# LiWentomng/OrientedRepPoints

Measured on NVIDIA H100. Metric: 1024x1024 tiles/sec, higher is better.
Workload: dtype f16x3

## Files before the change

### orientedreppoints_b200/csrc/dense_tc.cu

```cuda
#include <cuda.h>
#include <cuda_bf16.h>
#include <cuda_fp16.h>

#include <mutex>
#include <type_traits>

#include "common.cuh"
#include "../../include/orp_b200_group.h"
#include "wgmma.cuh"

namespace orp {
namespace {

constexpr int kMaxProb = 5;
constexpr int kStagesMax = 6;
constexpr int kBM = 128;
constexpr int kBK = 64;
constexpr int kABytes = kBM * kBK * 2;

struct FastDiv {
    uint32_t mul, shr, d;
    __host__ void set(uint32_t div)
    {
        d = div;
        uint32_t l = 0;
        while ((1ull << l) < div) ++l;
        shr = l;
        mul = (uint32_t)(((1ull << 32) * ((1ull << l) - div)) / div + 1);
    }
    __device__ __forceinline__ uint32_t div(uint32_t n) const { return (__umulhi(n, mul) + n) >> shr; }
    __device__ __forceinline__ void divmod(uint32_t n, uint32_t &q, uint32_t &r) const { q = div(n); r = n - q * d; }
};

struct Problem {
    int N, H, W, Ho, Wo;
    FastDiv fd_tw, fd_th;
    int BW, BH, BI;
    int lbw, lbh;
    int tiles_w, tiles_h, tiles_i, tile_start;
    void *out;
    const __nv_bfloat16 *res;
    const float *res32;
    const __nv_bfloat16 *x;
    const float *offset;
    const float *mask;
    double *gn_stats;
};

struct alignas(64) TcParams {
    CUtensorMap tmA[kMaxProb];
    CUtensorMap tmB;
    CUtensorMap tmOut[kMaxProb];
    CUtensorMap tmRes[kMaxProb];
    CUtensorMap tmI;
    Problem prob[kMaxProb];
    int tma_epi, epi_bufs;
    int epi_merge;
    int ncat;
    int ksplit;
    FastDiv fd_ks;
    long long ks_stride;
    int b_resident;
    int res_mma;
    int gn_fused;
    int dcat;
    int split;
    float oscale;
    unsigned int *ovf;
    int nprob, num_m_tiles, n_tiles_n, num_tiles;
    FastDiv fd_ntn;
    int KH, KW, Cin, cin_blocks, stride, pad, Cout, relu;
    int s2d_stem;
    const float *bias;
    int gw;
};

__device__ __forceinline__ uint32_t smem_u32(const void *p) { return (uint32_t)__cvta_generic_to_shared(p); }

__device__ __forceinline__ void mbar_init(uint64_t *bar, uint32_t count)
{
    asm volatile("mbarrier.init.shared::cta.b64 [%0], %1;" ::"r"(smem_u32(bar)), "r"(count));
}
__device__ __forceinline__ void mbar_expect_tx(uint64_t *bar, uint32_t bytes)
{
    asm volatile("mbarrier.arrive.expect_tx.shared::cta.b64 _, [%0], %1;" ::"r"(smem_u32(bar)), "r"(bytes) : "memory");
}
// ... 907 lines not shown
                                const float vy = wv.x * f1.y + wv.y * f2.y + wv.z * f3.y + wv.w * f4.y;
                                __nv_bfloat162 b2 = __floats2bfloat162_rn(vx, vy);
                                pk[k] = *reinterpret_cast<uint32_t *>(&b2);
                            }
                            *reinterpret_cast<uint4 *>(sa + (size_t)row * 128 + ((c16 ^ (row & 7)) << 4)) = make_uint4(pk[0], pk[1], pk[2], pk[3]);
                        }
                        asm volatile("fence.proxy.async.shared::cta;" ::: "memory");
                        __syncwarp();
                        if ((pt & 31) == 0) mbar_arrive(&full[r.stage]);
                        r.next();
                    } else {
                        const __half *xh = reinterpret_cast<const __half *>(pr.x);
                        auto load_item = [&](int it, uint4 (&u)[4][2]) {
                            const int item = pt + it * kDP, row = item >> 3, c16 = item & 7;
                            const int4 ov = s_o[tb][row];
                            const int co = cb * kBK + c16 * 8;
                            const int oo[4] = {ov.x, ov.y, ov.z, ov.w};
#pragma unroll
                            for (int c = 0; c < 4; ++c) {
                                u[c][0] = *reinterpret_cast<const uint4 *>(xh + oo[c] + co);
                                u[c][1] = *reinterpret_cast<const uint4 *>(xh + oo[c] + P.Cin + co);
                            }
                        };
                        auto item_at = [&](int it) {
                            const int item = pt + it * kDP, row = item >> 3, c16 = item & 7;
                            return (uint32_t)(row * 128 + ((c16 ^ (row & 7)) << 4));
                        };
                        if constexpr (!kFragEpi) {
                            uint32_t phi[kDItems][4], plo[kDItems][4];
#pragma unroll
                            for (int i2 = 0; i2 < kDItems / kDRound; ++i2) {
                                uint4 u[kDRound][4][2];
#pragma unroll
                                for (int i1 = 0; i1 < kDRound; ++i1) load_item(i2 * kDRound + i1, u[i1]);
#pragma unroll
                                for (int i1 = 0; i1 < kDRound; ++i1) {
                                    const int it = i2 * kDRound + i1, row = (pt + it * kDP) >> 3;
                                    split_sample(u[i1], s_w[tb][row], s_wh[tb][row], phi[it], plo[it]);
                                }
                            }
                            mbar_wait(&empty[r.stage], r.phase ^ 1);
                            if (pt == 0) load_b(r.stage, tap, cb, nt);
                            uint8_t *sa = smem + (size_t)r.stage * kStageBytes;
#pragma unroll
                            for (int it = 0; it < kDItems; ++it) {
                                const uint32_t at = item_at(it);
                                *reinterpret_cast<uint4 *>(sa + at) = make_uint4(phi[it][0], phi[it][1], phi[it][2], phi[it][3]);
                                *reinterpret_cast<uint4 *>(sa + kABytes + at) = make_uint4(plo[it][0], plo[it][1], plo[it][2], plo[it][3]);
                            }
                        } else {
                            const uint32_t sa = smem_u32(smem + (size_t)r.stage * kStageBytes);
#pragma unroll
                            for (int i2 = 0; i2 < kDItems / kDRound; ++i2) {
                                uint4 u[kDRound][4][2];
#pragma unroll
                                for (int i1 = 0; i1 < kDRound; ++i1) load_item(i2 * kDRound + i1, u[i1]);
                                if (i2 == 0) {
                                    mbar_wait(&empty[r.stage], r.phase ^ 1);
                                    if (pt == 0) load_b(r.stage, tap, cb, nt);
                                }
#pragma unroll
                                for (int i1 = 0; i1 < kDRound; ++i1) {
                                    const int it = i2 * kDRound + i1, row = (pt + it * kDP) >> 3;
                                    uint32_t hi[4], lo[4];
                                    split_sample(u[i1], s_w[tb][row], s_wh[tb][row], hi, lo);
                                    const uint32_t at = sa + item_at(it);
                                    sts128(at, make_uint4(hi[0], hi[1], hi[2], hi[3]));
                                    sts128(at + kABytes, make_uint4(lo[0], lo[1], lo[2], lo[3]));
                                }
                            }
                        }
                        asm volatile("fence.proxy.async.shared::cta;" ::: "memory");
                        __syncwarp();
                        if ((pt & 31) == 0) mbar_arrive(&full[r.stage]);
                        r.next();
                    }
                }
                tb ^= 1;
            }
        }
    }
}

typedef CUresult (*EncodeTiledFn)(CUtensorMap *, CUtensorMapDataType, cuuint32_t, void *, const cuuint64_t *, const cuuint64_t *,
                                  const cuuint32_t *, const cuuint32_t *, CUtensorMapInterleave, CUtensorMapSwizzle,
                                  CUtensorMapL2promotion, CUtensorMapFloatOOBfill);

EncodeTiledFn encode_fn()
{
    static EncodeTiledFn fn = nullptr;
    static std::once_flag once;
    std::call_once(once, [] {
        void *p = nullptr;
        cudaDriverEntryPointQueryResult st;
        if (cudaGetDriverEntryPoint("cuTensorMapEncodeTiled", &p, cudaEnableDefault, &st) == cudaSuccess && st == cudaDriverEntryPointSuccess)
            fn = reinterpret_cast<EncodeTiledFn>(p);
    });
    return fn;
}

int pow2_floor(int v) { int p = 1; while (p * 2 <= v) p *= 2; return p; }

constexpr int kEvPool = 1024;
thread_local cudaEvent_t g_tc_ev[kEvPool][2];
thread_local int g_tc_ev_created = 0, g_tc_ev_used = 0;
thread_local double g_tc_flops = 0.0;
thread_local orp_tc_plan g_tc_plan;
thread_local bool g_tc_plan_set = false;

constexpr int kSmemPerBlock = 227 * 1024;
constexpr int kStaticSmemPlain = 4096;
constexpr int kStaticSmemDeform = 14336;

struct ConvDesc {
    int nprob;
    const orp_tc_problem *probs;
    const void *w;
    int Cout, Cout_padded, KH, KW, Cin, stride, pad;
    const float *bias;
    int relu, out_f32, deform;
    int split;
    int wscale_log2;
    int stem;
    int ksplit;
    int gw;
};

struct ConvPlan {
    orp_tc_plan rep;
    Problem prob[kMaxProb];
    int num_m_tiles;
    int kbn;
    int extra_bytes;
};

int check_conv(const ConvDesc &d)
{
    if (d.split && (d.wscale_log2 < 0 || d.wscale_log2 > 15)) return fail(ORP_EINVAL, "conv2d_f16x3: weight scale exponent must be in 0..15");
    if (d.nprob < 1 || d.nprob > kMaxProb || !d.probs || !d.w) return fail(ORP_EINVAL, "conv2d_tc: bad arguments");
    if (d.Cin % 8) return fail(ORP_EINVAL, "conv2d_tc: Cin must be a multiple of 8 (16-byte channel rows)");
    if (d.deform && (d.Cin % kBK)) return fail(ORP_EINVAL, "conv2d_tc: deformable conv needs Cin % 64 == 0");
    if (d.Cout_padded % 32 || d.Cout_padded < d.Cout) return fail(ORP_EINVAL, "conv2d_tc: padded Cout must be a multiple of 32");
    if (d.stride < 1 || d.stride > 256) return fail(ORP_EINVAL, "conv2d_tc: stride must be in 1..256");
    if (d.deform)
        for (int i = 0; i < d.nprob; ++i)
            if ((long long)d.probs[i].N * d.probs[i].H * d.probs[i].W * d.Cin * (d.split ? 2 : 1) >= (1LL << 31))
                return fail(ORP_EINVAL, "conv2d_tc: deformable input has 2^31 or more 16-bit elements (32-bit sample offsets)");
    const orp_tc_problem &q0 = d.probs[0];
    if (d.ksplit > 1 && (d.nprob != 1 || d.deform || d.stem || !d.out_f32 || (d.KH * d.KW) % d.ksplit || q0.residual_bf16 ||
                         q0.residual_f32 || d.bias || d.relu))
        return fail(ORP_EINVAL, "conv2d_tc: split-K serves one plain problem with an fp32 partial-sum output and taps % ksplit == 0");
    if (d.gw) {
        if (d.gw != 4 && d.gw != 8 && d.gw != 16 && d.gw != 32 && d.gw != 64)
            return fail(ORP_EINVAL, "group_conv2d: group width (width / groups) must be 4, 8, 16, 32 or 64");
        if (d.Cout % kBK || d.Cin != d.Cout || d.Cout_padded != d.Cout)
            return fail(ORP_EINVAL, "group_conv2d: width must be a multiple of 64");
        if (d.nprob != 1 || d.out_f32 || d.deform || d.stem || d.ksplit != 1 || d.relu == 2 || d.KH != 3 || d.KW != 3 || d.pad != 1 ||
            q0.residual_bf16 || q0.residual_f32 || q0.offset || q0.mask || q0.gn_stats)
            return fail(ORP_EINVAL, "group_conv2d: one 3x3 / pad 1 problem with a 16-bit output; no residual, fp32 output, GroupNorm "
                                    "statistics, deformation or split-K");
    }
    return ORP_OK;
}

int plan_conv(const ConvDesc &d, int sms, ConvPlan &pl)
{
// ... 56 lines not shown
    int epi_bufs = mem_bound ? 2 : 1;
    const int epi_merge = (d.split && tma_epi && !frag_epi && (mem_bound || d.stem == 2)) ? 1 : 0;
    const int dcat = (d.split && d.deform) ? 1 : 0;
    const int ncat = (d.split && tma_epi && BN <= 128 && !d.deform && !any_res && !d.gw) ? 1 : 0;
    const int res_mma = (tma_epi && any_res) ? 1 : 0;
    if (res_mma) {
        if (d.deform) return fail(ORP_EINVAL, "conv2d_tc: residual is not supported on the deformable path");
        for (int i = 0; i < nprob; ++i)
            if (!probs[i].residual_bf16) return fail(ORP_EINVAL, "conv2d_tc: residual must be given for every problem or none");
    }
    const int slab_bytes = d.KH * d.KW * T * cin_blocks * BN * kBK * 2;
    int b_resident = (!d.deform && ksplit == 1 && slab_bytes <= 72 * 1024) ? 1 : 0;
    int grid = num_tiles / n_pair < sms ? num_tiles / n_pair : sms;
    if (b_resident && grid >= n_tiles_n) grid -= grid % n_tiles_n;
    else if (b_resident) b_resident = 0;
    int stage_b = 0, extra = 0, stages = 0;
    for (;;) {
        stage_b = stage_bytes(kbn, ncat || dcat, b_resident);
        const int hc = BN < 64 ? BN : 64;
        int staging = d.out_f32 ? 0 : 128 * (hc * 2 + 16);
        if (tma_epi) staging = epi_bufs * (epi_merge ? 32768 : 16384);
        extra = (res_mma ? 8192 : 0) + (b_resident ? slab_bytes : 0) + staging;
        stages = (kSmemPerBlock - (d.deform ? kStaticSmemDeform : kStaticSmemPlain) - dyn_smem_bytes(stage_b, 0, extra, frag_epi)) / stage_b;
        if (stages >= 3) break;
        if (epi_bufs == 2) { epi_bufs = 1; continue; }
        if (b_resident) { b_resident = 0; continue; }
        if (stages >= 2) break;
        return fail(ORP_EINVAL, "conv2d_tc: shared-memory budget cannot hold two main-loop stages");
    }
    if (stages > kStagesMax) stages = kStagesMax;
    if (d.deform && stages > 3) stages = 3;

    pl.num_m_tiles = mt;
    pl.kbn = kbn;
    pl.extra_bytes = extra;
    orp_tc_plan &r = pl.rep;
    r.BN = BN; r.stages = stages; r.grid = grid; r.num_tiles = num_tiles; r.n_tiles_n = n_tiles_n;
    r.ksplit = ksplit; r.nprob = nprob; r.Cout = d.Cout; r.Cout_padded = d.Cout_padded;
    r.split = d.split ? 1 : 0; r.deform = d.deform ? 1 : 0; r.out_f32 = d.out_f32 ? 1 : 0; r.stem = d.stem; r.relu = d.relu;
    r.bias = d.bias ? 1 : 0;
    for (int i = 0; i < nprob; ++i) {
        if (probs[i].residual_bf16) r.residual = 1;
        else if (probs[i].residual_f32) r.residual = 2;
        r.BW[i] = pl.prob[i].BW; r.BH[i] = pl.prob[i].BH; r.BI[i] = pl.prob[i].BI;
    }
    r.tma_epi = tma_epi; r.ncat = ncat; r.dcat = dcat; r.res_mma = res_mma; r.b_resident = b_resident;
    r.epi_merge = epi_merge; r.epi_bufs = epi_bufs; r.gn_fused = gn_fused; r.n_pair = n_pair;
    return ORP_OK;
}

int make_params(const ConvDesc &d, const ConvPlan &pl, TcParams &P)
{
    memset(&P, 0, sizeof(P));
    P.nprob = d.nprob; P.KH = d.KH; P.KW = d.KW; P.Cin = d.Cin; P.cin_blocks = d.gw ? 1 : (d.Cin + kBK - 1) / kBK;
    P.gw = d.gw;
    P.stride = d.stride; P.pad = d.pad;
    P.Cout = d.Cout; P.relu = d.relu; P.bias = d.bias; P.s2d_stem = (d.stem == 2) ? 1 : 0;
    P.split = d.split ? 1 : 0;
    P.oscale = d.split ? ldexpf(1.f, -d.wscale_log2) : 1.f;
    {
        void *ovf = nullptr;
        ORP_CUDA(cudaGetSymbolAddress(&ovf, g_f16_overflow));
        P.ovf = static_cast<unsigned int *>(ovf);
    }
    P.n_tiles_n = pl.rep.n_tiles_n / pl.rep.n_pair;
    P.fd_ntn.set((uint32_t)P.n_tiles_n);
    for (int i = 0; i < d.nprob; ++i) {
        const orp_tc_problem &q = d.probs[i];
        Problem &pr = P.prob[i];
        pr = pl.prob[i];
        pr.out = q.out; pr.res = static_cast<const __nv_bfloat16 *>(q.residual_bf16); pr.res32 = q.residual_f32;
        pr.x = static_cast<const __nv_bfloat16 *>(q.x); pr.offset = q.offset; pr.gn_stats = q.gn_stats; pr.mask = q.mask;
    }
    P.num_m_tiles = pl.num_m_tiles;
    P.num_tiles = pl.rep.num_tiles / pl.rep.n_pair;
    P.ksplit = d.ksplit;
    P.fd_ks.set((uint32_t)d.ksplit);
    P.ks_stride = (long long)P.prob[0].N * P.prob[0].Ho * P.prob[0].Wo * d.Cout;
    P.tma_epi = pl.rep.tma_epi; P.epi_bufs = pl.rep.epi_bufs; P.epi_merge = pl.rep.epi_merge; P.ncat = pl.rep.ncat;
    P.b_resident = pl.rep.b_resident; P.res_mma = pl.rep.res_mma; P.gn_fused = pl.rep.gn_fused; P.dcat = pl.rep.dcat;
    return ORP_OK;
}

int encode_maps(const ConvDesc &d, const ConvPlan &pl, TcParams &P)
{
    EncodeTiledFn enc = encode_fn();
    if (!enc) return fail(ORP_ECUDA, "conv2d_tc: cuTensorMapEncodeTiled unavailable");
    const CUtensorMapDataType dt16 = d.split ? CU_TENSOR_MAP_DATA_TYPE_FLOAT16 : CU_TENSOR_MAP_DATA_TYPE_BFLOAT16;
    const int T = d.split ? 2 : 1, Cin = d.Cin, Cout = d.Cout, stride = d.stride;
    if (!d.deform) {
        for (int i = 0; i < d.nprob; ++i) {
            const orp_tc_problem &q = d.probs[i];
            const Problem &pr = P.prob[i];
            cuuint64_t gdim[5] = {(cuuint64_t)Cin, (cuuint64_t)T, (cuuint64_t)q.W, (cuuint64_t)q.H, (cuuint64_t)q.N};
            cuuint64_t gstr[4] = {(cuuint64_t)Cin * 2, (cuuint64_t)Cin * 2 * T, (cuuint64_t)q.W * Cin * 2 * T,
                                  (cuuint64_t)q.H * q.W * Cin * 2 * T};
            if (d.stem == 2) {
                gstr[0] = (cuuint64_t)q.N * q.H * (q.W + 3) * 32;
                gstr[1] = 32;
                gstr[2] = (cuuint64_t)(q.W + 3) * 32;
                gstr[3] = (cuuint64_t)q.H * (q.W + 3) * 32;
            }
            cuuint32_t box[5] = {(cuuint32_t)kBK, 1u, (cuuint32_t)(pr.BW * stride), (cuuint32_t)(pr.BH * stride), (cuuint32_t)pr.BI};
            cuuint32_t estr[5] = {1, 1, (cuuint32_t)stride, (cuuint32_t)stride, 1};
            CUresult r = enc(&P.tmA[i], dt16, 5, const_cast<void *>(q.x), gdim, gstr, box, estr,
                             CU_TENSOR_MAP_INTERLEAVE_NONE, CU_TENSOR_MAP_SWIZZLE_128B, CU_TENSOR_MAP_L2_PROMOTION_L2_128B,
                             CU_TENSOR_MAP_FLOAT_OOB_FILL_NONE);
            if (r != CUDA_SUCCESS) return fail(ORP_ECUDA, "conv2d_tc: cuTensorMapEncodeTiled(A) failed");
        }
    }
    {
        const cuuint64_t K = (cuuint64_t)d.KH * d.KW * T * P.cin_blocks * kBK;
        cuuint64_t gdim[2] = {K, (cuuint64_t)d.Cout_padded};
        cuuint64_t gstr[1] = {K * 2};
        cuuint32_t box[2] = {(cuuint32_t)kBK, (cuuint32_t)pl.kbn};
        cuuint32_t estr[2] = {1, 1};
        CUresult r = enc(&P.tmB, dt16, 2, const_cast<void *>(d.w), gdim, gstr, box, estr,
                         CU_TENSOR_MAP_INTERLEAVE_NONE, CU_TENSOR_MAP_SWIZZLE_128B, CU_TENSOR_MAP_L2_PROMOTION_L2_256B,
                         CU_TENSOR_MAP_FLOAT_OOB_FILL_NONE);
        if (r != CUDA_SUCCESS) return fail(ORP_ECUDA, "conv2d_tc: cuTensorMapEncodeTiled(B) failed");
    }
    if (P.res_mma) {
        void *ident_ptr = nullptr;
        if (d.split) {
            ORP_CUDA(cudaGetSymbolAddress(&ident_ptr, g_ident16));
            ident_ptr = static_cast<char *>(ident_ptr) + (size_t)d.wscale_log2 * 8192;
        } else {
            ORP_CUDA(cudaGetSymbolAddress(&ident_ptr, g_ident));
        }
        cuuint64_t gdim[2] = {64, 64};
        cuuint64_t gstr[1] = {128};
        cuuint32_t box[2] = {64, 64};
        cuuint32_t estr[2] = {1, 1};
        CUresult r = enc(&P.tmI, dt16, 2, ident_ptr, gdim, gstr, box, estr, CU_TENSOR_MAP_INTERLEAVE_NONE,
                         CU_TENSOR_MAP_SWIZZLE_128B, CU_TENSOR_MAP_L2_PROMOTION_NONE, CU_TENSOR_MAP_FLOAT_OOB_FILL_NONE);
        if (r != CUDA_SUCCESS) return fail(ORP_ECUDA, "conv2d_tc: cuTensorMapEncodeTiled(identity) failed");
    }
    if (P.tma_epi) {
        for (int i = 0; i < d.nprob; ++i) {
            const Problem &pr = P.prob[i];
            cuuint64_t gdim[5] = {(cuuint64_t)Cout, (cuuint64_t)T, (cuuint64_t)pr.Wo, (cuuint64_t)pr.Ho, (cuuint64_t)pr.N};
            cuuint64_t gstr[4] = {(cuuint64_t)Cout * 2, (cuuint64_t)Cout * 2 * T, (cuuint64_t)pr.Wo * Cout * 2 * T,
                                  (cuuint64_t)pr.Ho * pr.Wo * Cout * 2 * T};
            cuuint32_t box[5] = {64u, 1u, (cuuint32_t)pr.BW, (cuuint32_t)pr.BH, (cuuint32_t)pr.BI};
            cuuint32_t estr[5] = {1, 1, 1, 1, 1};
            CUresult r = enc(&P.tmOut[i], dt16, 5, pr.out, gdim, gstr, box, estr,
                             CU_TENSOR_MAP_INTERLEAVE_NONE, CU_TENSOR_MAP_SWIZZLE_128B, CU_TENSOR_MAP_L2_PROMOTION_NONE,
                             CU_TENSOR_MAP_FLOAT_OOB_FILL_NONE);
            if (r != CUDA_SUCCESS) return fail(ORP_ECUDA, "conv2d_tc: cuTensorMapEncodeTiled(out) failed");
            if (pr.res) {
                r = enc(&P.tmRes[i], dt16, 5, const_cast<__nv_bfloat16 *>(pr.res), gdim, gstr, box, estr,
                        CU_TENSOR_MAP_INTERLEAVE_NONE, CU_TENSOR_MAP_SWIZZLE_128B, CU_TENSOR_MAP_L2_PROMOTION_L2_128B,
                        CU_TENSOR_MAP_FLOAT_OOB_FILL_NONE);
                if (r != CUDA_SUCCESS) return fail(ORP_ECUDA, "conv2d_tc: cuTensorMapEncodeTiled(residual) failed");
            }
        }
    }
    return ORP_OK;
}

template <int BN, bool OUT_F32, bool DEFORM, bool SPLIT, int WALK>
int launch_tc(const TcParams &P, int stages, int grid, cudaStream_t st, int extra_bytes)
{
    constexpr bool kCat = WALK == kWalkNcat || WALK == kWalkDcat;
    const int smem = dyn_smem_bytes(stage_bytes(BN, kCat, P.b_resident), stages, extra_bytes, frag_epilogue(BN, DEFORM));
    auto kern = conv_tc_kernel<BN, OUT_F32, DEFORM, SPLIT, WALK>;
    static int smem_max = -1;
    if (smem_max < 0) {
        cudaFuncAttributes fa;
        ORP_CUDA(cudaFuncGetAttributes(&fa, kern));
        ORP_CUDA(cudaFuncSetAttribute(kern, cudaFuncAttributeMaxDynamicSharedMemorySize, kSmemPerBlock - (int)fa.sharedSizeBytes));
        smem_max = kSmemPerBlock - (int)fa.sharedSizeBytes;
    }
    if (smem > smem_max) {
        char need[32];
        snprintf(need, sizeof(need), "%d", smem);
        return fail(ORP_EINVAL, "conv2d_tc: the plan's %s bytes of dynamic shared memory do not fit beside the static shared memory of %s",
                    need, __PRETTY_FUNCTION__);
    }
    int slot = -1;
    if (g_timing && g_tc_ev_used < kEvPool) {
        slot = g_tc_ev_used++;
        if (slot >= g_tc_ev_created) {
            ORP_CUDA(cudaEventCreate(&g_tc_ev[slot][0]));
            ORP_CUDA(cudaEventCreate(&g_tc_ev[slot][1]));
            g_tc_ev_created = slot + 1;
        }
        ORP_CUDA(cudaEventRecord(g_tc_ev[slot][0], st));
        double fl = 0;
        for (int i = 0; i < P.nprob; ++i)
            fl += 2.0 * P.prob[i].N * P.prob[i].Ho * P.prob[i].Wo * (double)P.Cout *
                  (P.s2d_stem ? 147.0 : (double)P.KH * P.KW * (P.gw ? P.gw : P.Cin));
        g_tc_flops += fl;
    }
    {
        cudaLaunchConfig_t cfg;
        memset(&cfg, 0, sizeof(cfg));
        cfg.gridDim = dim3((unsigned)grid);
        cfg.blockDim = dim3(DEFORM ? (unsigned)(kConsumers + kDP) : (unsigned)(kConsumers + 128));
        cfg.dynamicSmemBytes = smem;
        cfg.stream = st;
        cudaLaunchAttribute at[1];
        at[0].id = cudaLaunchAttributeProgrammaticStreamSerialization;
        at[0].val.programmaticStreamSerializationAllowed = 1;
        cfg.attrs = at;
        cfg.numAttrs = 1;
        ORP_CUDA(cudaLaunchKernelEx(&cfg, kern, P, stages));
    }
    ORP_LAUNCHED();
    if (slot >= 0) ORP_CUDA(cudaEventRecord(g_tc_ev[slot][1], st));
    return ORP_OK;
}

template <int BN, bool OUT_F32, bool DEFORM>
int launch_plan(const TcParams &P, int stages, int grid, cudaStream_t st, int extra_bytes)
{
    if constexpr (DEFORM) {
        if (P.dcat != P.split || P.ncat || P.res_mma) return fail(ORP_EINVAL, "conv2d_tc: deformable plan outside dcat == split");
        if constexpr (frag_epilogue(BN, true)) {
            if (!P.split || OUT_F32 || !P.tma_epi || P.epi_merge || P.gn_fused || P.relu == 2)
                return fail(ORP_EINVAL, "conv2d_tc: deformable N-tile pair outside f16x3 with an unmerged TMA epilogue and no GELU");
            return launch_tc<BN, false, true, true, kWalkDcat>(P, stages, grid, st, extra_bytes);
        } else {
            return P.split ? launch_tc<BN, OUT_F32, true, true, kWalkDcat>(P, stages, grid, st, extra_bytes)
                           : launch_tc<BN, OUT_F32, true, false, kWalkK>(P, stages, grid, st, extra_bytes);
        }
    } else {
        if (P.gw) {
            if constexpr (BN == 64 && !OUT_F32) {
                if (P.ncat || P.res_mma) return fail(ORP_EINVAL, "group_conv2d: grouped plan with ncat or a residual");
                if (P.gw <= 16)
                    return P.split ? launch_tc<64, false, false, true, kWalkG16>(P, stages, grid, st, extra_bytes)
                                   : launch_tc<64, false, false, false, kWalkG16>(P, stages, grid, st, extra_bytes);
                if (P.gw == 32)
                    return P.split ? launch_tc<64, false, false, true, kWalkG32>(P, stages, grid, st, extra_bytes)
                                   : launch_tc<64, false, false, false, kWalkG32>(P, stages, grid, st, extra_bytes);
                return P.split ? launch_tc<64, false, false, true, kWalkG64>(P, stages, grid, st, extra_bytes)
                               : launch_tc<64, false, false, false, kWalkG64>(P, stages, grid, st, extra_bytes);
            }
            return fail(ORP_EINVAL, "group_conv2d: grouped plan outside BN 64 with a 16-bit output");
        }
        if (P.ncat && P.res_mma) return fail(ORP_EINVAL, "conv2d_tc: ncat plan with a residual");
        if (P.ncat) {
            if constexpr (!OUT_F32 && BN >= 64 && BN <= 128) {
                if (P.split) return launch_tc<BN, false, false, true, kWalkNcat>(P, stages, grid, st, extra_bytes);
            }
            return fail(ORP_EINVAL, "conv2d_tc: ncat plan outside f16x3 TMA-epilogue layers with BN 64..128");
        }
        if (P.res_mma) {
            if constexpr (!OUT_F32 && BN >= 64)
                return P.split ? launch_tc<BN, false, false, true, kWalkKRes>(P, stages, grid, st, extra_bytes)
                               : launch_tc<BN, false, false, false, kWalkKRes>(P, stages, grid, st, extra_bytes);
            return fail(ORP_EINVAL, "conv2d_tc: residual K blocks outside TMA-epilogue layers with BN >= 64");
        }
        return P.split ? launch_tc<BN, OUT_F32, false, true, kWalkK>(P, stages, grid, st, extra_bytes)
                       : launch_tc<BN, OUT_F32, false, false, kWalkK>(P, stages, grid, st, extra_bytes);
    }
}

template <bool OUT_F32, bool DEFORM>
int launch_bn(const TcParams &P, const ConvPlan &pl, cudaStream_t st)
{
    const int s = pl.rep.stages, g = pl.rep.grid, e = pl.extra_bytes;
    switch (pl.kbn) {
    case 256:
        if constexpr (!DEFORM || !OUT_F32) return launch_plan<256, OUT_F32, DEFORM>(P, s, g, st, e);
        break;
    case 128: return launch_plan<128, OUT_F32, DEFORM>(P, s, g, st, e);
    case 64: return launch_plan<64, OUT_F32, DEFORM>(P, s, g, st, e);
    case 32: return launch_plan<32, OUT_F32, DEFORM>(P, s, g, st, e);
    }
    return fail(ORP_EINVAL, "conv2d_tc: unsupported tile width");
}

int conv2d_tc(const ConvDesc &d, void *stream)
{
    int rc = check_conv(d);
    if (rc) return rc;
    rc = ensure_device();
    if (rc) return rc;
    int sms = 0;
    rc = device_sms(sms);
    if (rc) return rc;
    ConvPlan pl;
    rc = plan_conv(d, sms, pl);
    if (rc) return rc;
    TcParams P;
    rc = make_params(d, pl, P);
    if (rc) return rc;
    rc = encode_maps(d, pl, P);
    if (rc) return rc;
    g_tc_plan = pl.rep;
    g_tc_plan_set = true;
    cudaStream_t st = static_cast<cudaStream_t>(stream);
    rc = d.out_f32 ? (d.deform ? launch_bn<true, true>(P, pl, st) : launch_bn<true, false>(P, pl, st))
                   : (d.deform ? launch_bn<false, true>(P, pl, st) : launch_bn<false, false>(P, pl, st));
    if (rc) return rc;
    bool want_gn = false;
    for (int i = 0; i < d.nprob; ++i) want_gn = want_gn || (d.probs[i].gn_stats != nullptr);
    if (want_gn && !P.gn_fused) {
        if (d.out_f32 || d.Cout != 256) return fail(ORP_EINVAL, "conv2d_tc: gn_stats needs a 16-bit output with 256 channels");
        for (int i = 0; i < d.nprob; ++i)
            if (d.probs[i].gn_stats) {
                int r2 = d.split ? orp_gn_stats_f16x3(P.prob[i].out, P.prob[i].N, P.prob[i].Ho * P.prob[i].Wo, 256, 32, d.probs[i].gn_stats, stream)
                                 : orp_gn_stats_bf16(P.prob[i].out, P.prob[i].N, P.prob[i].Ho * P.prob[i].Wo, 256, 32, d.probs[i].gn_stats, stream);
                if (r2) return r2;
            }
    }
    return ORP_OK;
}

int stem_desc(const void *x_s2d, int N, int H, int W, const void *w, const float *bias, int relu, void *out, int split,
              int wscale_log2, orp_tc_problem &q, ConvDesc &d)
{
    if (!x_s2d || !w || !out || N < 1 || H < 2 || W < 2 || (H & 1) || (W & 1))
        return fail(ORP_EINVAL, "stem_conv_s2d_%s: needs even H, W", split ? "f16x3" : "bf16");
    if (split && (wscale_log2 < 0 || wscale_log2 > 15)) return fail(ORP_EINVAL, "stem_conv_s2d_f16x3: weight scale exponent must be in 0..15");
    memset(&q, 0, sizeof(q));
    q.x = x_s2d;
    q.N = N; q.H = H / 2 + 3; q.W = W / 2; q.out = out;
    d = ConvDesc{1, &q, w, 64, 64, 4, 1, 64, 1, 0, bias, relu, 0, 0, split, split ? wscale_log2 : 0, 2, 1};
    return ORP_OK;
}

int splitk_desc(const orp_tc_problem *prob, const void *w, int Cout, int Cout_padded, int KH, int KW, int Cin, int stride, int pad,
                int f16x3, int wscale_log2, int ksplit, void *workspace, orp_tc_problem &q, ConvDesc &d, int &Ho, int &Wo)
{
    if (!prob || !w || !workspace || ksplit < 2 || (Cout % 8)) return fail(ORP_EINVAL, "conv2d_tc_splitk: bad arguments");
    if (f16x3 && (wscale_log2 < 0 || wscale_log2 > 15)) return fail(ORP_EINVAL, "conv2d_tc_splitk: weight scale exponent must be in 0..15");
    Ho = (prob->H + 2 * pad - (KH - 1) - 1) / stride + 1;
    Wo = (prob->W + 2 * pad - (KW - 1) - 1) / stride + 1;
    if (Ho <= 0 || Wo <= 0) return fail(ORP_EINVAL, "conv2d_tc_splitk: bad problem");
    q = *prob;
    q.out = workspace;
    q.gn_stats = nullptr;
    d = ConvDesc{1, &q, w, Cout, Cout_padded, KH, KW, Cin, stride, pad, nullptr, 0, 1, 0, f16x3 ? 1 : 0, wscale_log2, 0, ksplit};
    return ORP_OK;
}

__global__ void __launch_bounds__(256)
splitk_finish_kernel(const float *__restrict__ ws, int ksplit, size_t pixels, int C, const float *__restrict__ bias, int relu, int split,
                     void *__restrict__ out, unsigned int *ovf)
{
    const int c8 = C / 8;
    const size_t total = pixels * c8;
    for (size_t i = blockIdx.x * (size_t)blockDim.x + threadIdx.x; i < total; i += (size_t)gridDim.x * blockDim.x) {
        const size_t pix = i / c8;
        const int c = (int)(i - pix * c8) * 8;
        float v[8] = {0.f, 0.f, 0.f, 0.f, 0.f, 0.f, 0.f, 0.f};
        for (int k = 0; k < ksplit; ++k) {
            const float *p = ws + (size_t)k * pixels * C + pix * C + c;
            const float4 a = *reinterpret_cast<const float4 *>(p), b = *reinterpret_cast<const float4 *>(p + 4);
            v[0] += a.x; v[1] += a.y; v[2] += a.z; v[3] += a.w; v[4] += b.x; v[5] += b.y; v[6] += b.z; v[7] += b.w;
        }
        float amax = 0.f;
#pragma unroll
        for (int j = 0; j < 8; ++j) {
            if (bias) v[j] += bias[c + j];
            if (relu) v[j] = fmaxf(v[j], 0.f);
            amax = fmaxf(amax, fabsf(v[j]));
        }
        uint32_t hi[4], lo[4];
        if (split) {
#pragma unroll
            for (int k = 0; k < 4; ++k) {
                const __half2 h2 = __floats2half2_rn(v[2 * k], v[2 * k + 1]);
                const float2 hf = __half22float2(h2);
                const __half2 l2 = __floats2half2_rn(v[2 * k] - hf.x, v[2 * k + 1] - hf.y);
                hi[k] = *reinterpret_cast<const uint32_t *>(&h2);
                lo[k] = *reinterpret_cast<const uint32_t *>(&l2);
            }
            __half *o = static_cast<__half *>(out) + pix * 2 * C + c;
            *reinterpret_cast<uint4 *>(o) = make_uint4(hi[0], hi[1], hi[2], hi[3]);
            *reinterpret_cast<uint4 *>(o + C) = make_uint4(lo[0], lo[1], lo[2], lo[3]);
            if (amax > 65504.f) atomicAdd(ovf, 1u);
        } else {
#pragma unroll
            for (int k = 0; k < 4; ++k) {
                __nv_bfloat162 b2 = __floats2bfloat162_rn(v[2 * k], v[2 * k + 1]);
                hi[k] = *reinterpret_cast<uint32_t *>(&b2);
            }
            *reinterpret_cast<uint4 *>(static_cast<__nv_bfloat16 *>(out) + pix * C + c) = make_uint4(hi[0], hi[1], hi[2], hi[3]);
        }
    }
}
}
}

using namespace orp;

extern "C" int orp_tc_timing_collect(float *total_ms, int *launches, double *flops)
{
    if (!total_ms || !launches || !flops) return fail(ORP_EINVAL, "orp_tc_timing_collect: null");
    float sum = 0.f;
    for (int i = 0; i < g_tc_ev_used; ++i) {
        float ms = 0.f;
        ORP_CUDA(cudaEventSynchronize(g_tc_ev[i][1]));
        ORP_CUDA(cudaEventElapsedTime(&ms, g_tc_ev[i][0], g_tc_ev[i][1]));
        sum += ms;
    }
    *total_ms = sum; *launches = g_tc_ev_used; *flops = g_tc_flops;
    g_tc_ev_used = 0; g_tc_flops = 0.0;
    return ORP_OK;
}

extern "C" int orp_tc_last_plan(orp_tc_plan *out)
{
    if (!out) return fail(ORP_EINVAL, "orp_tc_last_plan: null");
    if (!g_tc_plan_set) return fail(ORP_EINVAL, "orp_tc_last_plan: no tensor-core convolution launched on this thread");
    *out = g_tc_plan;
    return ORP_OK;
}

extern "C" int orp_tc_plan_conv(int nprob, const orp_tc_problem *probs, const void *w, int Cout, int Cout_padded, int KH, int KW,
                                int Cin, int stride, int pad, const float *bias, int wscale_log2, int relu, int out_f32, int deform,
                                int split, int stem, int ksplit, int sms, orp_tc_plan *out)
{
    if (!out || sms < 1 || (stem != 0 && stem != 2)) return fail(ORP_EINVAL, "orp_tc_plan_conv: bad arguments");
    split = split ? 1 : 0;
    orp_tc_problem q;
    ConvDesc d;
    int rc = ORP_OK;
    if (stem == 2 || ksplit > 1) {
        if (nprob != 1 || !probs || deform || out_f32 || (stem == 2 && ksplit > 1))
            return fail(ORP_EINVAL, "orp_tc_plan_conv: the stem and split-K plan one problem with a 16-bit output");
        int Ho, Wo;
        rc = stem == 2 ? stem_desc(probs->x, probs->N, probs->H, probs->W, w, bias, relu, probs->out, split, wscale_log2, q, d)
                       : splitk_desc(probs, w, Cout, Cout_padded, KH, KW, Cin, stride, pad, split, wscale_log2, ksplit, probs->out, q,
                                     d, Ho, Wo);
    } else {
        d = ConvDesc{nprob, probs, w, Cout, Cout_padded, KH, KW, Cin, stride, pad, bias, relu, out_f32, deform, split, wscale_log2, 0, 1};
    }
    if (rc) return rc;
    ConvPlan pl;
    rc = plan_conv(d, sms, pl);
    if (rc) return rc;
    *out = pl.rep;
    return ORP_OK;
}

extern "C" int orp_conv2d_bf16(int nprob, const orp_tc_problem *probs, const void *w, int Cout, int Cout_padded, int KH,
                               int KW, int Cin, int stride, int pad, const float *bias, int relu, int out_f32,
                               int deform, void *stream)
{
    return conv2d_tc(ConvDesc{nprob, probs, w, Cout, Cout_padded, KH, KW, Cin, stride, pad, bias, relu, out_f32, deform, 0, 0, 0, 1},
                     stream);
}

extern "C" int orp_conv2d_f16x3(int nprob, const orp_tc_problem *probs, const void *w_split, int Cout, int Cout_padded, int KH,
                                int KW, int Cin, int stride, int pad, const float *bias, int wscale_log2, int relu,
                                int out_f32, int deform, void *stream)
{
    return conv2d_tc(ConvDesc{nprob, probs, w_split, Cout, Cout_padded, KH, KW, Cin, stride, pad, bias, relu, out_f32, deform, 1,
                              wscale_log2, 0, 1},
                     stream);
}

ConvDesc group_desc(const orp_tc_problem *probs, int nprob, const void *w, int width, int groups, int stride, const float *bias,
                    int relu, int out_f32, int split, int wscale_log2)
{
    const int gw = (groups >= 1 && width % groups == 0) ? width / groups : -1;
    return ConvDesc{nprob, probs, w, width, width, 3, 3, width, stride, 1, bias, relu, out_f32, 0, split, split ? wscale_log2 : 0, 0,
                    1, gw};
}

extern "C" int orp_group_conv2d_bf16(const orp_tc_problem *prob, const void *w, int width, int groups, int stride, const float *bias,
                                     int relu, void *stream)
{
    return conv2d_tc(group_desc(prob, 1, w, width, groups, stride, bias, relu, 0, 0, 0), stream);
}

extern "C" int orp_group_conv2d_f16x3(const orp_tc_problem *prob, const void *w_split, int width, int groups, int stride,
                                      const float *bias, int wscale_log2, int relu, void *stream)
{
    return conv2d_tc(group_desc(prob, 1, w_split, width, groups, stride, bias, relu, 0, 1, wscale_log2), stream);
}

extern "C" int orp_tc_plan_group_conv(int nprob, const orp_tc_problem *probs, const void *w, int width, int groups, int stride,
                                      const float *bias, int relu, int out_f32, int split, int sms, orp_tc_plan *out)
{
    if (!out || sms < 1) return fail(ORP_EINVAL, "orp_tc_plan_group_conv: bad arguments");
    ConvPlan pl;
    const int rc = plan_conv(group_desc(probs, nprob, w, width, groups, stride, bias, relu, out_f32, split ? 1 : 0, 0), sms, pl);
    if (rc) return rc;
    *out = pl.rep;
    return ORP_OK;
}
// ... 75 lines not shown
```

Baseline: 322.3.

## Add streamed half-tile 1x1 conv kernel for f16x3 256-column tiles

Adds a specialized kernel for 1x1 f16x3 convolutions that loads A in half-tile (64-row) slots, one per consumer warpgroup. This gives a deeper ring of smaller stages, so each warpgroup can start its MMAs and epilogue without waiting for the full 128-row tile and the two groups' work is staggered via named barriers. TMA boxes for input and output are halved, and the output store writes the hi/lo split pair in one 2-deep box. It is enabled by default for eligible plans, adds a sizeable separate code path, and carries a risk of synchronization or phase bugs.

```diff
diff --git a/orientedreppoints_b200/csrc/dense_tc.cu b/orientedreppoints_b200/csrc/dense_tc.cu
--- a/orientedreppoints_b200/csrc/dense_tc.cu
+++ b/orientedreppoints_b200/csrc/dense_tc.cu
@@ -2,6 +2,7 @@
 #include <cuda_bf16.h>
 #include <cuda_fp16.h>
 
+#include <atomic>
 #include <mutex>
 #include <type_traits>
 
@@ -1075,6 +1076,258 @@
     }
 }
 
+
+__host__ __device__ __forceinline__ void half_box(int BW, int BH, int BI, int h, int &dw, int &dh, int &di)
+{
+    dw = dh = di = 0;
+    if (BI > 1) di = h * (BI >> 1);
+    else if (BH > 1) dh = h * (BH >> 1);
+    else dw = h * (BW >> 1);
+}
+
+constexpr int kMaxHalfStages = 16;
+
+template <int BN, int WALK>
+__global__ void __launch_bounds__(kConsumers + 128, 1)
+conv_tc_kernel_1x1_stream(const __grid_constant__ TcParams P, int stages)
+{
+    static_assert(BN == 256 && (WALK == kWalkK || WALK == kWalkKRes), "streamed 1x1: f16x3, 256-column tiles, K-concatenated walk");
+    constexpr int kHalfA = kABytes / 2;
+    constexpr int kBBytes = BN * kBK * 2;
+    constexpr int kSlot = 16384;
+    extern __shared__ __align__(1024) uint8_t smem_raw[];
+    uint8_t *smem = reinterpret_cast<uint8_t *>((reinterpret_cast<uintptr_t>(smem_raw) + 1023) & ~uintptr_t(1023));
+    uint8_t *ident = smem;
+    if (P.res_mma) smem += 8192;
+    const int kblocks_all = P.cin_blocks * 2;
+    uint8_t *bres = smem;
+    if (P.b_resident) smem += (size_t)kblocks_all * kBBytes;
+    uint8_t *ring = smem;
+    const int ring_bytes = kAccBytes + stages * stage_bytes(BN, false, P.b_resident);
+    uint8_t *stage_out = smem + ring_bytes;
+    const int half_bytes = kHalfA + (P.b_resident ? 0 : kBBytes);
+    const int nslots = min(ring_bytes / half_bytes, kMaxHalfStages);
+    __shared__ uint64_t full[kMaxHalfStages], empty[kMaxHalfStages];
+    __shared__ uint64_t bres_bar;
+
+    const int warp = threadIdx.x >> 5, lane = threadIdx.x & 31;
+    if (warp == kConsumers / 32 && elect_one()) {
+        asm volatile("prefetch.tensormap [%0];" ::"l"(&P.tmA[0]) : "memory");
+        asm volatile("prefetch.tensormap [%0];" ::"l"(&P.tmB) : "memory");
+    }
+    if (warp == 0) {
+        if (elect_one()) {
+            for (int s = 0; s < nslots; ++s) {
+                mbar_init(&full[s], 1);
+                mbar_init(&empty[s], 1);
+            }
+            mbar_init(&bres_bar, 1);
+            asm volatile("fence.mbarrier_init.release.cluster;" ::: "memory");
+        }
+        __syncwarp();
+    }
+    __syncthreads();
+    const int kblocks = P.cin_blocks * 3;
+    auto res_groups_of = [&](int nt) {
+        int n = 0;
+        if constexpr (WALK == kWalkKRes)
+            for (int g = 0; g < BN / 64 && nt * BN + g * 64 < P.Cout; ++g) ++n;
+        return n;
+    };
+    auto nt_of = [&](int tile) { return tile - (int)P.fd_ntn.div((uint32_t)tile) * P.n_tiles_n; };
+    asm volatile("griddepcontrol.launch_dependents;" ::: "memory");
+    asm volatile("griddepcontrol.wait;" ::: "memory");
+
+    if (warp < kConsumers / 32) {
+        setmaxnreg_inc<kConsumerRegs>();
+        const int g = warp >> 2;
+        const bool leader = (threadIdx.x & 127) == 0;
+        const int frow = (warp & 3) * 16 + (lane >> 2), fcol = 2 * (lane & 3);
+        auto bar_sync = [](int id, int n) { asm volatile("bar.sync %0, %1;" ::"r"(id), "r"(n) : "memory"); };
+        auto bar_arrive = [](int id, int n) { asm volatile("bar.arrive %0, %1;" ::"r"(id), "r"(n) : "memory"); };
+        if ((P.b_resident || P.res_mma) && (int)blockIdx.x < P.num_tiles) mbar_wait(&bres_bar, 0);
+        const uint32_t obuf = smem_u32(stage_out) + (uint32_t)(g * P.epi_bufs * kSlot);
+        int ob = 0;
+        float acc[BN / 2];
+        uint32_t base = 0;
+        for (int tile = blockIdx.x, k = 0; tile < P.num_tiles; tile += gridDim.x, ++k) {
+            const int nt = nt_of(tile), res_groups = res_groups_of(nt);
+            const int unit = kblocks + 2 * res_groups;
+            const uint32_t pos = base + (uint32_t)(g * unit);
+            base += 2u * (uint32_t)unit;
+            if (g == 1) bar_sync(2, kConsumers);
+            else if (k > 0) bar_sync(3, kConsumers);
+            int slot = (int)(pos % (uint32_t)nslots);
+            uint32_t phase = (pos / (uint32_t)nslots) & 1u;
+            auto advance = [&]() { if (++slot == nslots) { slot = 0; phase ^= 1u; } };
+            int held = -1;
+            auto release = [&](int next) {
+                if (held >= 0 && leader) mbar_arrive(&empty[held]);
+                held = next;
+            };
+            KIter it(1, P.cin_blocks, 1, 0);
+            for (int kb = 0; kb < kblocks; ++kb, it.next()) {
+                mbar_wait(&full[slot], phase);
+                const uint32_t sa = smem_u32(ring + (size_t)slot * half_bytes);
+                const uint64_t da = make_desc_sw128(sa);
+                const uint64_t db = make_desc_sw128(P.b_resident ? smem_u32(bres + (size_t)(it.cb * 2 + (it.term == 2 ? 1 : 0)) * kBBytes)
+                                                                 : sa + kHalfA);
+                wgmma_fence();
+#pragma unroll
+                for (int k16 = 0; k16 < kBK / 16; ++k16) {
+                    if constexpr (WALK == kWalkKRes)
+                        wgmma_cols64<BN / 64, false>(acc, da + (uint64_t)(k16 * 2), db + (uint64_t)(k16 * 2), (kb | k16) ? 1u : 0u);
+                    else
+                        wgmma_n<BN, false>(acc, da + (uint64_t)(k16 * 2), db + (uint64_t)(k16 * 2), (kb | k16) ? 1u : 0u);
+                }
+                wgmma_commit();
+                wgmma_wait<1>();
+                release(slot);
+                advance();
+            }
+            if constexpr (WALK == kWalkKRes) {
+                wgmma_wait<0>();
+                release(-1);
+                auto res_group = [&](auto gc) {
+                    constexpr int G = decltype(gc)::value;
+                    if (G >= res_groups) return;
+#pragma unroll 1
+                    for (int t = 0; t < 2; ++t) {
+                        mbar_wait(&full[slot], phase);
+                        const uint64_t da = make_desc_sw128(smem_u32(ring + (size_t)slot * half_bytes));
+                        const uint64_t db = make_desc_sw128(smem_u32(ident));
+                        wgmma_fence();
+#pragma unroll
+                        for (int k16 = 0; k16 < kBK / 16; ++k16)
+                            wgmma_n<64, false>(acc_view<32 * G, 32>(acc), da + (uint64_t)(k16 * 2), db + (uint64_t)(k16 * 2), 1u);
+                        wgmma_commit();
+                        wgmma_wait<1>();
+                        release(slot);
+                        advance();
+                    }
+                };
+                res_group(std::integral_constant<int, 0>{});
+                res_group(std::integral_constant<int, 1>{});
+                res_group(std::integral_constant<int, 2>{});
+                res_group(std::integral_constant<int, 3>{});
+            }
+            if (g == 0) bar_arrive(2, kConsumers);
+            else if (tile + (int)gridDim.x < P.num_tiles) bar_arrive(3, kConsumers);
+            wgmma_wait<0>();
+            wgmma_fence_acc(acc);
+            release(-1);
+
+            int pi, wb, hb, ib, ntt;
+            decode_tile(P, tile, pi, wb, hb, ib, ntt);
+            const Problem &pr = P.prob[pi];
+            int dw, dh, di;
+            half_box(pr.BW, pr.BH, pr.BI, g, dw, dh, di);
+            bool valid_r[2];
+#pragma unroll
+            for (int hr = 0; hr < 2; ++hr) {
+                const int r = 64 * g + frow + 8 * hr;
+                const int iw = r & (pr.BW - 1), ih = (r >> pr.lbw) & (pr.BH - 1), ii = r >> (pr.lbw + pr.lbh);
+                valid_r[hr] = (wb * pr.BW + iw < pr.Wo) && (hb * pr.BH + ih < pr.Ho) && (ib * pr.BI + ii < pr.N);
+            }
+            float amax[2][2] = {{0.f, 0.f}, {0.f, 0.f}};
+#pragma unroll
+            for (int G = 0; G < BN / 64; ++G) {
+                if (leader) {
+                    if (P.epi_bufs == 2) asm volatile("cp.async.bulk.wait_group.read 1;" ::: "memory");
+                    else asm volatile("cp.async.bulk.wait_group.read 0;" ::: "memory");
+                }
+                bar_sync(4 + g, 128);
+                const uint32_t obase = obuf + (uint32_t)ob * (uint32_t)kSlot;
+#pragma unroll
+                for (int i = 0; i < 8; ++i) {
+                    const int c = G * 8 + i;
+                    const int col = nt * BN + c * 8 + fcol;
+                    const float2 bv = (P.bias && col < P.Cout) ? *reinterpret_cast<const float2 *>(P.bias + col) : make_float2(0.f, 0.f);
+#pragma unroll
+                    for (int hr = 0; hr < 2; ++hr) {
+                        float f0 = acc[4 * c + 2 * hr], f1 = acc[4 * c + 2 * hr + 1];
+                        f0 *= P.oscale; f1 *= P.oscale;
+                        f0 += bv.x; f1 += bv.y;
+                        if (P.relu == 1) { f0 = fmaxf(f0, 0.f); f1 = fmaxf(f1, 0.f); }
+                        amax[hr][i >> 2] = fmaxf(fmaxf(amax[hr][i >> 2], fabsf(f0)), fabsf(f1));
+                        const __half2 h2 = __floats2half2_rn(f0, f1);
+                        const float2 hf = __half22float2(h2);
+                        const __half2 l2 = __floats2half2_rn(f0 - hf.x, f1 - hf.y);
+                        const uint32_t r2 = 2u * (uint32_t)(frow + 8 * hr);
+                        const uint32_t ah = obase + r2 * 128u + ((uint32_t)(i ^ (r2 & 7)) << 4) + (uint32_t)fcol * 2u;
+                        const uint32_t al = obase + (r2 + 1u) * 128u + ((uint32_t)(i ^ ((r2 + 1u) & 7)) << 4) + (uint32_t)fcol * 2u;
+                        asm volatile("st.shared.b32 [%0], %1;" ::"r"(ah), "r"(*reinterpret_cast<const uint32_t *>(&h2)) : "memory");
+                        asm volatile("st.shared.b32 [%0], %1;" ::"r"(al), "r"(*reinterpret_cast<const uint32_t *>(&l2)) : "memory");
+                    }
+                }
+                asm volatile("fence.proxy.async.shared::cta;" ::: "memory");
+                bar_sync(4 + g, 128);
+                if (leader) {
+                    asm volatile(
+                        "cp.async.bulk.tensor.5d.global.shared::cta.bulk_group [%0, {%2, %3, %4, %5, %6}], [%1];"
+                        ::"l"(&P.tmOut[pi]), "r"(obase), "r"(nt * BN + G * 64), "r"(0),
+                          "r"(wb * pr.BW + dw), "r"(hb * pr.BH + dh), "r"(ib * pr.BI + di) : "memory");
+                    asm volatile("cp.async.bulk.commit_group;" ::: "memory");
+                }
+                if (++ob == P.epi_bufs) ob = 0;
+            }
+#pragma unroll
+            for (int hr = 0; hr < 2; ++hr)
+#pragma unroll
+                for (int hc = 0; hc < 2; ++hc) {
+                    float m = amax[hr][hc];
+                    m = fmaxf(m, __shfl_xor_sync(0xffffffffu, m, 1));
+                    m = fmaxf(m, __shfl_xor_sync(0xffffffffu, m, 2));
+                    if ((lane & 3) == 0 && valid_r[hr] && m > 65504.f) atomicAdd(P.ovf, 1u);
+                }
+        }
+        if (leader) asm volatile("cp.async.bulk.wait_group 0;" ::: "memory");
+    } else {
+        setmaxnreg_dec<kProducerRegs>();
+        if (warp == kConsumers / 32 && elect_one()) {
+            if ((P.b_resident || P.res_mma) && (int)blockIdx.x < P.num_tiles) {
+                mbar_expect_tx(&bres_bar, (uint32_t)((P.b_resident ? kblocks_all * kBBytes : 0) + (P.res_mma ? 8192 : 0)));
+                if (P.res_mma) tma_load_2d(ident, &P.tmI, &bres_bar, 0, 0);
+                if (P.b_resident)
+                    for (int kb = 0; kb < kblocks_all; ++kb)
+                        tma_load_2d(bres + (size_t)kb * kBBytes, &P.tmB, &bres_bar, kb * kBK, nt_of(blockIdx.x) * BN);
+            }
+            int slot = 0;
+            uint32_t phase = 0;
+            auto next = [&]() { if (++slot == nslots) { slot = 0; phase ^= 1u; } };
+            for (int tile = blockIdx.x; tile < P.num_tiles; tile += gridDim.x) {
+                int pi, wb, hb, ib, nt;
+                decode_tile(P, tile, pi, wb, hb, ib, nt);
+                const Problem &pr = P.prob[pi];
+                const int res_groups = res_groups_of(nt);
+                for (int h = 0; h < 2; ++h) {
+                    int dw, dh, di;
+                    half_box(pr.BW, pr.BH, pr.BI, h, dw, dh, di);
+                    const int w0 = (wb * pr.BW + dw) * P.stride - P.pad, h0 = (hb * pr.BH + dh) * P.stride - P.pad, i0 = ib * pr.BI + di;
+                    KIter it(1, P.cin_blocks, 1, 0);
+                    for (int j = 0; j < kblocks; ++j, it.next()) {
+                        mbar_wait(&empty[slot], phase ^ 1u);
+                        uint8_t *sa = ring + (size_t)slot * half_bytes;
+                        mbar_expect_tx(&full[slot], half_bytes);
+                        tma_load_5d(sa, &P.tmA[pi], &full[slot], it.cb * kBK, it.term == 1 ? 1 : 0, w0, h0, i0);
+                        if (!P.b_resident)
+                            tma_load_2d(sa + kHalfA, &P.tmB, &full[slot], (it.cb * 2 + (it.term == 2 ? 1 : 0)) * kBK, nt * BN);
+                        next();
+                    }
+                    for (int rg = 0; rg < res_groups; ++rg)
+                        for (int t = 0; t < 2; ++t) {
+                            mbar_wait(&empty[slot], phase ^ 1u);
+                            mbar_expect_tx(&full[slot], kHalfA);
+                            tma_load_5d(ring + (size_t)slot * half_bytes, &P.tmRes[pi], &full[slot], nt * BN + rg * 64, t,
+                                        wb * pr.BW + dw, hb * pr.BH + dh, ib * pr.BI + di);
+                            next();
+                        }
+                }
+            }
+        }
+    }
+}
+
 typedef CUresult (*EncodeTiledFn)(CUtensorMap *, CUtensorMapDataType, cuuint32_t, void *, const cuuint64_t *, const cuuint64_t *,
                                   const cuuint32_t *, const cuuint32_t *, CUtensorMapInterleave, CUtensorMapSwizzle,
                                   CUtensorMapL2promotion, CUtensorMapFloatOOBfill);
@@ -1297,7 +1550,23 @@
     return ORP_OK;
 }
 
-int encode_maps(const ConvDesc &d, const ConvPlan &pl, TcParams &P)
+void half_box_dims(int &bw, int &bh, int &bi)
+{
+    int dw, dh, di;
+    half_box(bw, bh, bi, 1, dw, dh, di);
+    bw -= dw; bh -= dh; bi -= di;
+}
+
+std::atomic<int> g_tc_staged_1x1{0};
+bool streams_1x1(const ConvDesc &d, const ConvPlan &pl)
+{
+    const orp_tc_plan &r = pl.rep;
+    return !g_tc_staged_1x1.load() && r.split && !r.deform && !r.out_f32 && !d.gw && !d.stem && r.ksplit == 1 && d.KH == 1 &&
+           d.KW == 1 && r.tma_epi && r.epi_merge && !r.gn_fused && !r.ncat && r.relu != 2 && pl.kbn == 256 &&
+           d.Cin <= 256 && (r.res_mma || !r.b_resident);
+}
+
+int encode_maps(const ConvDesc &d, const ConvPlan &pl, TcParams &P, bool stream)
 {
     EncodeTiledFn enc = encode_fn();
     if (!enc) return fail(ORP_ECUDA, "conv2d_tc: cuTensorMapEncodeTiled unavailable");
@@ -1316,7 +1585,9 @@
                 gstr[2] = (cuuint64_t)(q.W + 3) * 32;
                 gstr[3] = (cuuint64_t)q.H * (q.W + 3) * 32;
             }
-            cuuint32_t box[5] = {(cuuint32_t)kBK, 1u, (cuuint32_t)(pr.BW * stride), (cuuint32_t)(pr.BH * stride), (cuuint32_t)pr.BI};
+            int bw = pr.BW, bh = pr.BH, bi = pr.BI;
+            if (stream) half_box_dims(bw, bh, bi);
+            cuuint32_t box[5] = {(cuuint32_t)kBK, 1u, (cuuint32_t)(bw * stride), (cuuint32_t)(bh * stride), (cuuint32_t)bi};
             cuuint32_t estr[5] = {1, 1, (cuuint32_t)stride, (cuuint32_t)stride, 1};
             CUresult r = enc(&P.tmA[i], dt16, 5, const_cast<void *>(q.x), gdim, gstr, box, estr,
                              CU_TENSOR_MAP_INTERLEAVE_NONE, CU_TENSOR_MAP_SWIZZLE_128B, CU_TENSOR_MAP_L2_PROMOTION_L2_128B,
@@ -1357,9 +1628,12 @@
             cuuint64_t gdim[5] = {(cuuint64_t)Cout, (cuuint64_t)T, (cuuint64_t)pr.Wo, (cuuint64_t)pr.Ho, (cuuint64_t)pr.N};
             cuuint64_t gstr[4] = {(cuuint64_t)Cout * 2, (cuuint64_t)Cout * 2 * T, (cuuint64_t)pr.Wo * Cout * 2 * T,
                                   (cuuint64_t)pr.Ho * pr.Wo * Cout * 2 * T};
-            cuuint32_t box[5] = {64u, 1u, (cuuint32_t)pr.BW, (cuuint32_t)pr.BH, (cuuint32_t)pr.BI};
+            int bw = pr.BW, bh = pr.BH, bi = pr.BI;
+            if (stream) half_box_dims(bw, bh, bi);
+            cuuint32_t box[5] = {64u, 1u, (cuuint32_t)bw, (cuuint32_t)bh, (cuuint32_t)bi};
+            cuuint32_t obox[5] = {64u, stream ? 2u : 1u, (cuuint32_t)bw, (cuuint32_t)bh, (cuuint32_t)bi};
             cuuint32_t estr[5] = {1, 1, 1, 1, 1};
-            CUresult r = enc(&P.tmOut[i], dt16, 5, pr.out, gdim, gstr, box, estr,
+            CUresult r = enc(&P.tmOut[i], dt16, 5, pr.out, gdim, gstr, obox, estr,
                              CU_TENSOR_MAP_INTERLEAVE_NONE, CU_TENSOR_MAP_SWIZZLE_128B, CU_TENSOR_MAP_L2_PROMOTION_NONE,
                              CU_TENSOR_MAP_FLOAT_OOB_FILL_NONE);
             if (r != CUDA_SUCCESS) return fail(ORP_ECUDA, "conv2d_tc: cuTensorMapEncodeTiled(out) failed");
@@ -1374,12 +1648,13 @@
     return ORP_OK;
 }
 
-template <int BN, bool OUT_F32, bool DEFORM, bool SPLIT, int WALK>
+template <int BN, bool OUT_F32, bool DEFORM, bool SPLIT, int WALK, bool STREAM = false>
 int launch_tc(const TcParams &P, int stages, int grid, cudaStream_t st, int extra_bytes)
 {
     constexpr bool kCat = WALK == kWalkNcat || WALK == kWalkDcat;
     const int smem = dyn_smem_bytes(stage_bytes(BN, kCat, P.b_resident), stages, extra_bytes, frag_epilogue(BN, DEFORM));
     auto kern = conv_tc_kernel<BN, OUT_F32, DEFORM, SPLIT, WALK>;
+    if constexpr (STREAM) kern = conv_tc_kernel_1x1_stream<BN, WALK>;
     static int smem_max = -1;
     if (smem_max < 0) {
         cudaFuncAttributes fa;
@@ -1428,8 +1703,14 @@
 }
 
 template <int BN, bool OUT_F32, bool DEFORM>
-int launch_plan(const TcParams &P, int stages, int grid, cudaStream_t st, int extra_bytes)
-{
+int launch_plan(const TcParams &P, int stages, int grid, cudaStream_t st, int extra_bytes, bool stream)
+{
+    if (stream) {
+        if constexpr (BN == 256 && !OUT_F32 && !DEFORM)
+            return P.res_mma ? launch_tc<256, false, false, true, kWalkKRes, true>(P, stages, grid, st, extra_bytes)
+                             : launch_tc<256, false, false, true, kWalkK, true>(P, stages, grid, st, extra_bytes);
+        return fail(ORP_EINVAL, "conv2d_tc: streamed 1x1 plan outside 256-column f16x3 tiles with a 16-bit output");
+    }
     if constexpr (DEFORM) {
         if (P.dcat != P.split || P.ncat || P.res_mma) return fail(ORP_EINVAL, "conv2d_tc: deformable plan outside dcat == split");
         if constexpr (frag_epilogue(BN, true)) {
@@ -1474,16 +1755,16 @@
 }
 
 template <bool OUT_F32, bool DEFORM>
-int launch_bn(const TcParams &P, const ConvPlan &pl, cudaStream_t st)
+int launch_bn(const TcParams &P, const ConvPlan &pl, cudaStream_t st, bool stream)
 {
     const int s = pl.rep.stages, g = pl.rep.grid, e = pl.extra_bytes;
     switch (pl.kbn) {
     case 256:
-        if constexpr (!DEFORM || !OUT_F32) return launch_plan<256, OUT_F32, DEFORM>(P, s, g, st, e);
+        if constexpr (!DEFORM || !OUT_F32) return launch_plan<256, OUT_F32, DEFORM>(P, s, g, st, e, stream);
         break;
-    case 128: return launch_plan<128, OUT_F32, DEFORM>(P, s, g, st, e);
-    case 64: return launch_plan<64, OUT_F32, DEFORM>(P, s, g, st, e);
-    case 32: return launch_plan<32, OUT_F32, DEFORM>(P, s, g, st, e);
+    case 128: return launch_plan<128, OUT_F32, DEFORM>(P, s, g, st, e, stream);
+    case 64: return launch_plan<64, OUT_F32, DEFORM>(P, s, g, st, e, stream);
+    case 32: return launch_plan<32, OUT_F32, DEFORM>(P, s, g, st, e, stream);
     }
     return fail(ORP_EINVAL, "conv2d_tc: unsupported tile width");
 }
@@ -1503,13 +1784,14 @@
     TcParams P;
     rc = make_params(d, pl, P);
     if (rc) return rc;
-    rc = encode_maps(d, pl, P);
+    const bool streamed = streams_1x1(d, pl);
+    rc = encode_maps(d, pl, P, streamed);
     if (rc) return rc;
     g_tc_plan = pl.rep;
     g_tc_plan_set = true;
     cudaStream_t st = static_cast<cudaStream_t>(stream);
-    rc = d.out_f32 ? (d.deform ? launch_bn<true, true>(P, pl, st) : launch_bn<true, false>(P, pl, st))
-                   : (d.deform ? launch_bn<false, true>(P, pl, st) : launch_bn<false, false>(P, pl, st));
+    rc = d.out_f32 ? (d.deform ? launch_bn<true, true>(P, pl, st, streamed) : launch_bn<true, false>(P, pl, st, streamed))
+                   : (d.deform ? launch_bn<false, true>(P, pl, st, streamed) : launch_bn<false, false>(P, pl, st, streamed));
     if (rc) return rc;
     bool want_gn = false;
     for (int i = 0; i < d.nprob; ++i) want_gn = want_gn || (d.probs[i].gn_stats != nullptr);
@@ -1618,6 +1900,8 @@
     g_tc_ev_used = 0; g_tc_flops = 0.0;
     return ORP_OK;
 }
+
+extern "C" void orp_test_tc_staged_1x1(int on) { g_tc_staged_1x1.store(on ? 1 : 0); }
 
 extern "C" int orp_tc_last_plan(orp_tc_plan *out)
 {
```

After: 327.1, median of 6. 1.5% higher.
